# smallflyingpig/speech-to-image-translation-without-text

Hardware: AMD Instinct MI355X
Metric: StackGAN-v2 3-stage G+D train-step images/sec at 256px (higher is better)
Workload: dtype f32

## Files before the change

speech_to_image_translation_without_text_amd/csrc/s2i_conv_fwd.hip:

```cpp
#include "s2i_igemm.h"

namespace {

__global__ __launch_bounds__(256) void split_packed_kernel(const float* __restrict__ src, unsigned short* __restrict__ dst_rc,
                                                           unsigned short* __restrict__ dst_cr, int R, int C, int NP,
                                                           long long plane) {
  __shared__ float tile[32][33];
  const int t = blockIdx.z;
  const int r0 = blockIdx.y * 32, c0 = blockIdx.x * 32;
  const int tx = threadIdx.x & 31, ty = threadIdx.x >> 5;
  const float* sp = src + (size_t)t * R * C;
#pragma unroll
  for (int k = 0; k < 4; ++k) {
    const int r = r0 + ty + 8 * k, c = c0 + tx;
    tile[ty + 8 * k][tx] = (r < R && c < C) ? sp[(size_t)r * C + c] : 0.f;
  }
  __syncthreads();
#pragma unroll
  for (int k = 0; k < 4; ++k) {
    if (dst_rc) {
      const int r = r0 + ty + 8 * k, c = c0 + tx;
      if (r < R && c < C) {
        float v = tile[ty + 8 * k][tx];
        const size_t o = ((size_t)t * R + r) * C + c;
        for (int pl = 0; pl < NP; ++pl) {
          const __bf16 h = (__bf16)v;
          dst_rc[pl * plane + o] = __builtin_bit_cast(unsigned short, h);
          v -= (float)h;
        }
      }
    }
    if (dst_cr) {
      const int c = c0 + ty + 8 * k, r = r0 + tx;
      if (r < R && c < C) {
        float v = tile[tx][ty + 8 * k];
        const size_t o = ((size_t)t * C + c) * R + r;
        for (int pl = 0; pl < NP; ++pl) {
          const __bf16 h = (__bf16)v;
          dst_cr[pl * plane + o] = __builtin_bit_cast(unsigned short, h);
          v -= (float)h;
        }
      }
    }
  }
}

template <int LPP>
__global__ __launch_bounds__(256) void small_n_conv_kernel(IgemmP p) {
  extern __shared__ __attribute__((aligned(16))) float wl[];
  constexpr int PPW = 64 / LPP;
  const int tid = threadIdx.x, lane = tid & 63, wave = tid >> 6;
  const int phase = blockIdx.z;
  const int py = phase >> 1, px = phase & 1;
  int s, pad, kw;
  geom(p.kind, p.g_s, p.g_pad, p.g_kw, s, pad, kw);
  for (int e = tid; e < p.T * p.Ca; e += 256) {
    const int t = e / p.Ca, c = e - t * p.Ca;
    const int tw = tap_weight(p.kind, p.flip, p.T, t, py, px);
    f32x4 v = {0.f, 0.f, 0.f, 0.f};
    if (p.wt) {
#pragma unroll
      for (int n = 0; n < 4; ++n)
        if (n < p.N) v[n] = p.w[((size_t)tw * p.wR + n) * p.ldw + c];
    } else {
#pragma unroll
      for (int n = 0; n < 4; ++n)
        if (n < p.N && n < p.ldw) v[n] = p.w[((size_t)tw * p.wR + c) * p.ldw + n];
    }
    *reinterpret_cast<f32x4*>(wl + e * 4) = v;
  }
  __syncthreads();
  const int q = lane % LPP, pl = lane / LPP;
  const int ngroups = (p.M + PPW - 1) / PPW;
  for (int grp = blockIdx.x * 4 + wave; grp < ngroups; grp += gridDim.x * 4) {
    const int m = grp * PPW + pl;
    f32x4 acc = {0.f, 0.f, 0.f, 0.f};
    int b = 0, oy = 0, ox = 0;
    if (m < p.M) {
      b = m >> p.lgHoWo;
      const int r = m & ((1 << p.lgHoWo) - 1);
      oy = r >> p.lgWo;
      ox = r & (p.Wo - 1);
      const int by = oy * s - pad, bx = ox * s - pad;
      const unsigned mask = tap_mask(p.kind, kw, by, bx, p.H, p.W, py, px);
      const long long xo = (((long long)b * p.H + by) * p.W + bx) * p.Cx + q * 4;
      for (int t = 0; t < p.T; ++t) {
        if (!((mask >> t) & 1u)) continue;
        int dy, dx;
        tap_delta(p.kind, kw, t, py, px, dy, dx);
        const long long xe = xo + ((long long)dy * p.W + dx) * p.Cx;
        f32x4 xv;
        if (p.x16) {
          const u32x2_t h = *reinterpret_cast<const u32x2_t*>(reinterpret_cast<const unsigned short*>(p.x) + xe);
          xv = f32x4{__builtin_bit_cast(float, h[0] << 16), __builtin_bit_cast(float, h[0] & 0xffff0000u),
                     __builtin_bit_cast(float, h[1] << 16), __builtin_bit_cast(float, h[1] & 0xffff0000u)};
        } else {
          xv = *reinterpret_cast<const f32x4*>(p.x + xe);
        }
        const float* wp = wl + ((size_t)t * p.Ca + q * 4) * 4;
#pragma unroll
        for (int j = 0; j < 4; ++j) acc += xv[j] * *reinterpret_cast<const f32x4*>(wp + j * 4);
      }
    }
#pragma unroll
    for (int sft = 1; sft < LPP; sft <<= 1)
#pragma unroll
      for (int n = 0; n < 4; ++n) acc[n] += __shfl_xor(acc[n], sft);
    if (q == 0 && m < p.M) {
      long long row = m;
      if (p.kind == S2I_TCONV_K4S2) row = ((long long)b * (2 * p.Ho) + 2 * oy + py) * (2 * p.Wo) + 2 * ox + px;
      f32x4 o;
#pragma unroll
      for (int n = 0; n < 4; ++n) {
        float v = acc[n];
        if (p.bias && n < p.N) v += p.bias[n];
        if (p.act == S2I_ACT_LRELU) v = v > 0.f ? v : 0.2f * v;
        else if (p.act == S2I_ACT_TANH) v = tanhf(v);
        else if (p.act == S2I_ACT_RELU) v = fmaxf(v, 0.f);
        o[n] = v;
      }
      if (p.N == 4 && !p.y16 && (p.ldy & 3) == 0) {
        *reinterpret_cast<f32x4*>(p.y + row * p.ldy) = o;
      } else {
#pragma unroll
        for (int n = 0; n < 4; ++n) {
          if (n >= p.N) break;
          if (p.y16) reinterpret_cast<unsigned short*>(p.y)[row * p.ldy + n] = f2bf(o[n]);
          else p.y[row * p.ldy + n] = o[n];
        }
      }
    }
  }
}

__global__ void splitk_reduce_kernel(const float* __restrict__ slab, int S, long long rows, int N,
                                     const float* __restrict__ bias, int act, float* __restrict__ y,
                                     int ldy, int y16) {
  const long long total = rows * N;
  for (long long e = (long long)blockIdx.x * blockDim.x + threadIdx.x; e < total;
       e += (long long)gridDim.x * blockDim.x) {
    const long long row = e / N;
    const int n = (int)(e - row * N);
    float v = 0.f;
    for (int s = 0; s < S; ++s) v += slab[(size_t)s * total + e];
    if (bias) v += bias[n];
    if (act == S2I_ACT_LRELU) v = v > 0.f ? v : 0.2f * v;
    else if (act == S2I_ACT_TANH) v = tanhf(v);
    else if (act == S2I_ACT_RELU) v = fmaxf(v, 0.f);
    if (y16) reinterpret_cast<unsigned short*>(y)[row * ldy + n] = f2bf(v);
    else y[row * ldy + n] = v;
  }
}

__global__ __launch_bounds__(256) void splitk_reduce_stats_kernel(const float* __restrict__ slab, int S, long long rows,
                                                                  int N, float* __restrict__ y, int ldy,
                                                                  float* __restrict__ part, int nparts, int cpb,
                                                                  int ppg, long long Rg, int y16) {
  __shared__ f32x4 sh[2][256];
  const int tid = threadIdx.x;
  const int rpb = 256 / cpb;
  const int ql = tid % cpb, rl = tid / cpb;
  const int quad = blockIdx.y * cpb + ql;
  const int Q = N / 4;
  const int grp = blockIdx.x / ppg, pp = blockIdx.x - grp * ppg;
  const long long chunk = (Rg + ppg - 1) / ppg;
  const long long r0 = grp * Rg + pp * chunk;
  const long long gend = (grp + 1) * Rg < rows ? (grp + 1) * Rg : rows;
  const long long r1 = r0 + chunk < gend ? r0 + chunk : gend;
  const size_t sstride = (size_t)rows * N;
  f32x4 s0 = {0.f, 0.f, 0.f, 0.f}, s1 = {0.f, 0.f, 0.f, 0.f};
  if (quad < Q) {
    for (long long row = r0 + rl; row < r1; row += rpb) {
      const float* sp = slab + row * N + quad * 4;
      f32x4 v = *reinterpret_cast<const f32x4*>(sp);
      for (int s = 1; s < S; ++s) v += *reinterpret_cast<const f32x4*>(sp + s * sstride);
      if (y16) {
        unsigned short* yp = reinterpret_cast<unsigned short*>(y) + row * ldy + quad * 4;
        *reinterpret_cast<u32x2_t*>(yp) = u32x2_t{(unsigned)f2bf(v[0]) | ((unsigned)f2bf(v[1]) << 16),
                                                 (unsigned)f2bf(v[2]) | ((unsigned)f2bf(v[3]) << 16)};
      } else {
        *reinterpret_cast<f32x4*>(y + row * ldy + quad * 4) = v;
      }
      s0 += v;
      s1 += v * v;
    }
  }
  sh[0][tid] = s0;
  sh[1][tid] = s1;
  __syncthreads();
  if (rl == 0 && quad < Q) {
    for (int r = 1; r < rpb; ++r) {
      s0 += sh[0][r * cpb + ql];
      s1 += sh[1][r * cpb + ql];
    }
    *reinterpret_cast<f32x4*>(part + ((size_t)0 * nparts + blockIdx.x) * N + quad * 4) = s0;
    *reinterpret_cast<f32x4*>(part + ((size_t)1 * nparts + blockIdx.x) * N + quad * 4) = s1;
  }
}

}

int launch_igemm_fwd(const FwdPlan& pl, const IgemmP& p, hipStream_t st) {
  const dim3 grid(pl.gx, pl.gy, pl.gz);
  switch (pl.kernel) {
    case FWD_F32_128x128: case FWD_F32IN_128x128: launch_fwd_128x128(pl, p, grid, st); break;
    case FWD_F32_128x64: case FWD_F32IN_128x64: launch_fwd_128x64(pl, p, grid, st); break;
    case FWD_F32_128x32: case FWD_F32IN_128x32: launch_fwd_128x32(pl, p, grid, st); break;
    case FWD_F32_96x128: case FWD_F32IN_96x128: launch_fwd_96x128(pl, p, grid, st); break;
    case FWD_SPLIT_128x128: case FWD_SPLIT_128x64: case FWD_SPLIT_128x32: launch_fwd_split(pl, p, grid, st); break;
    default: S2I_FAIL("igemm_fwd: kernel %d is no matrix kernel", (int)pl.kernel);
  }
  S2I_LAUNCH_CHECK("igemm_fwd");
  return 0;
}

int launch_small_n_conv(const FwdPlan& pl, const IgemmP& p, hipStream_t st) {
  const dim3 grid(pl.gx, pl.gy, pl.gz);
  const size_t shb = (size_t)pl.T * pl.Ca * 4 * sizeof(float);
  if (pl.kernel == FWD_SMALLN_4) hipLaunchKernelGGL((small_n_conv_kernel<4>), grid, dim3(256), shb, st, p);
  else if (pl.kernel == FWD_SMALLN_8) hipLaunchKernelGGL((small_n_conv_kernel<8>), grid, dim3(256), shb, st, p);
  else hipLaunchKernelGGL((small_n_conv_kernel<16>), grid, dim3(256), shb, st, p);
  S2I_LAUNCH_CHECK("small_n_conv");
  return 0;
}

int launch_splitk_reduce(const s2i_conv_desc* d, const FwdPlan& pl, const float* bias, float* y, float* part, void* ws,
                         int y16, void* stream) {
  hipStream_t st = (hipStream_t)stream;
  if (pl.reduce == FWD_REDUCE_STATS) {
    const int Q = d->N / 4;
    int cpb = 1;
    while (cpb < Q && cpb < 256) cpb <<= 1;
    const int groups = d->groups < 1 ? 1 : d->groups;
    const int nparts = stat_parts(pl, groups);
    hipLaunchKernelGGL(splitk_reduce_stats_kernel, dim3(nparts, (Q + cpb - 1) / cpb), dim3(256), 0, st,
                       (const float*)ws, pl.splitk, pl.Mrows, d->N, y, d->ldy, part, nparts, cpb, nparts / groups,
                       pl.Mrows / groups, y16);
    S2I_LAUNCH_CHECK("splitk_reduce_stats");
    return 0;
  }
  const long long total = pl.Mrows * d->N;
  int blocks = s2i_cdiv(total, 256);
  if (blocks > 4096) blocks = 4096;
  hipLaunchKernelGGL(splitk_reduce_kernel, dim3(blocks), dim3(256), 0, st, (const float*)ws, pl.splitk,
                     pl.Mrows, d->N, bias, d->act, y, d->ldy, y16);
  S2I_LAUNCH_CHECK("splitk_reduce");
  if (pl.reduce == FWD_REDUCE_COLSTATS) return s2i_colstats(y, pl.Mrows, d->N, d->ldy, part, stat_parts(pl, 1), stream);
  return 0;
}

extern "C" int s2i_split_packed_weight(const float* packed, int T, int R, int C, int planes, unsigned short* out_rc,
                                       unsigned short* out_cr, void* stream) {
  S2I_REQUIRE(packed && (out_rc || out_cr) && T > 0 && R > 0 && C > 0 && planes >= 1 && planes <= 3,
              "split_packed_weight: bad args");
  dim3 grid(s2i_cdiv(C, 32), s2i_cdiv(R, 32), T);
  hipLaunchKernelGGL(split_packed_kernel, grid, dim3(256), 0, (hipStream_t)stream, packed, out_rc, out_cr, R, C, planes,
                     (long long)T * R * C);
  S2I_LAUNCH_CHECK("split_packed_weight");
  return 0;
}
```

speech_to_image_translation_without_text_amd/csrc/s2i_wgrad.hip:

```cpp
#include "s2i_igemm.h"

namespace {

struct WgradP {
  const float* __restrict__ a;
  const float* __restrict__ cvec;
  const float* __restrict__ g;
  float* __restrict__ slab;
  int B, H, W, Ca, Cc, Cin;
  int Ho, Wo, lgWo, lgHoWo;
  int M, N, ldg, K, T, kind;
  int cps, nchunks;
  int a16, g16;
  unsigned a_bytes, c_bytes, g_bytes;
  const float* __restrict__ a_coef;
  int a_groups, a_ipg;
};

__device__ __forceinline__ bool wgrad_col(const WgradP& p, int kcol, int kw, int& c, int& dy, int& dx) {
  c = 0;
  dy = 0;
  dx = 0;
  if (kcol >= p.K) return false;
  const int t = kcol / p.Cin;
// ... 285 lines not shown
  geom(p.kind, 1, 0, 1, s, pad, kw);
  const int acol8 = tid % ATPR, arow = tid / ATPR;
  const int bcol8 = tid % BTPR, brow = tid / BTPR;
  int c, dy, dx;
  const bool kvalid = wgrad_col(p, k0 + acol8 * 8, kw, c, dy, dx);
  const int nb = n0 + bcol8 * 8;
  const bool nvalid = nb < p.N;
  const __amdgpu_buffer_rsrc_t ra_rs = __builtin_amdgcn_make_buffer_rsrc((void*)p.a, 0, p.a_bytes, 0x00020000);
  const __amdgpu_buffer_rsrc_t rg_rs = __builtin_amdgcn_make_buffer_rsrc((void*)p.g, 0, p.g_bytes, 0x00020000);
  u32x4 ra[APASS], rb[BPASS];
  auto fetch = [&](int pc) {
#pragma unroll
    for (int q = 0; q < APASS; ++q) {
      const int m = pc * PC + arow + q * AROWS;
      int b, oy, ox;
      row_pixel(p, m, b, oy, ox);
      const int iy = oy * s - pad + dy, ix = ox * s - pad + dx;
      if constexpr (A32) {
        const bool rowok = kvalid && m < p.M && iy >= 0 && iy < p.H;
        const int o0 = ((b * p.H + iy) * p.W + ix) * 16;
        const f32x4 v0 = bload4(ra_rs, (rowok && ix >= 0 && ix < p.W) ? o0 : S2I_OOB);
        const f32x4 v1 = bload4(ra_rs, (rowok && ix + 1 >= 0 && ix + 1 < p.W) ? o0 + 16 : S2I_OOB);
        ra[q] = u32x4{(unsigned)f2bf(v0[0]) | ((unsigned)f2bf(v0[1]) << 16), (unsigned)f2bf(v0[2]) | ((unsigned)f2bf(v0[3]) << 16),
                      (unsigned)f2bf(v1[0]) | ((unsigned)f2bf(v1[1]) << 16), (unsigned)f2bf(v1[2]) | ((unsigned)f2bf(v1[3]) << 16)};
      } else {
        const bool ok = kvalid && m < p.M && iy >= 0 && iy < p.H && ix >= 0 && ix < p.W;
        ra[q] = __builtin_amdgcn_raw_buffer_load_b128(ra_rs, ok ? (((b * p.H + iy) * p.W + ix) * p.Ca + c) * 2 : S2I_OOB, 0, 0);
      }
    }
#pragma unroll
    for (int q = 0; q < BPASS; ++q) {
      const int row = brow + q * BROWS;
      const int m = pc * PC + row;
      rb[q] = __builtin_amdgcn_raw_buffer_load_b128(rg_rs, (row < PC && m < p.M && nvalid) ? (m * p.ldg + nb) * 2 : S2I_OOB, 0, 0);
    }
  };

  f32x16 acc[TM][TN];
  zero_acc(acc);

  int aad[TM][2], bad[TN][2];
  wgrad_tr_addr<TM, AROWB>(lane, wm, aad);
  wgrad_tr_addr<TN, BROWB>(lane, wn, bad);

  const int c_begin = split * p.cps;
  const int c_end = min(p.nchunks, c_begin + p.cps);
  auto stage_store = [&](unsigned char* A_, unsigned char* B_) {
#pragma unroll
    for (int q = 0; q < APASS; ++q) {
      const int row = arow + q * AROWS;
      const int sw = ((row & 3) << 2) | ((row >> 2) & 3);
      *reinterpret_cast<u32x4*>(A_ + row * AROWB + 16 * ((acol8 ^ sw) & AMASK)) = ra[q];
    }
#pragma unroll
    for (int q = 0; q < BPASS; ++q) {
      const int row = brow + q * BROWS;
      const int sw = ((row & 3) << 2) | ((row >> 2) & 3);
      if (row < PC) *reinterpret_cast<u32x4*>(B_ + row * BROWB + 16 * ((bcol8 ^ sw) & BMASK)) = rb[q];
    }
  };
  auto stage_mma = [&](const unsigned char* A_, const unsigned char* B_) {
#pragma unroll
    for (int ks = 0; ks < PC / 16; ++ks) {
      bf16x8 a[TM], b[TN];
#pragma unroll
      for (int i = 0; i < TM; ++i) a[i] = lds_tr_frag(A_ + ks * 16 * AROWB, aad[i]);
#pragma unroll
      for (int j = 0; j < TN; ++j) b[j] = lds_tr_frag(B_ + ks * 16 * BROWB, bad[j]);
#pragma unroll
      for (int i = 0; i < TM; ++i)
#pragma unroll
        for (int j = 0; j < TN; ++j)
          acc[i][j] = __builtin_amdgcn_mfma_f32_32x32x16_bf16(a[i], b[j], acc[i][j], 0, 0, 0);
    }
  };
  if (c_begin < c_end) fetch(c_begin);
  for (int pc = c_begin; pc < c_end; ++pc) {
    stage_store(As, Bs);
    __syncthreads();
    if (pc + 1 < c_end) fetch(pc + 1);
    stage_mma(As, Bs);
    __syncthreads();
  }

  store_wgrad_slab<TM, TN>(p, split, k0, n0, acc, lane, wm, wn);
}

template <int CIN, int BN, int WAVES_M, int WAVES_N, int DYS>
__global__ __launch_bounds__(64 * WAVES_M * WAVES_N, 3) void wgrad_k3_rows_kernel(WgradP p) {
  constexpr int NT = 64 * WAVES_M * WAVES_N;
  constexpr int BM = 3 * CIN * DYS, RT = BM / 32;
  constexpr int TM = RT / WAVES_M, TN = BN / (32 * WAVES_N);
  static_assert(TM * WAVES_M == RT && TN * WAVES_N * 32 == BN, "tile split");
  constexpr int LDH = CIN, LDB = BN;
  constexpr int CQ = CIN / 4, HQR = 34 * CQ, HQ = DYS * HQR;
  constexpr int HPASS = (HQ + NT - 1) / NT;
  constexpr int BROWS = NT * 4 / BN, BPASS = (32 + BROWS - 1) / BROWS;
  static_assert(BROWS * BN == NT * 4, "a pass must cover whole rows");
  __shared__ __attribute__((aligned(16))) float smem[DYS * 34 * LDH + 32 * LDB];
  float* Hs = smem;
  float* Bs = smem + DYS * 34 * LDH;
  const int tid = threadIdx.x, lane = tid & 63, wave = tid >> 6;
  const int wm = wave / WAVES_N, wn = wave % WAVES_N;
  const int dy0 = DYS == 3 ? 0 : blockIdx.x, n0 = blockIdx.y * BN, split = blockIdx.z;
  const int bcol4 = tid % (BN / 4), brow = tid / (BN / 4);
  const int nb = n0 + bcol4 * 4;
  const int gcolb = nb < p.N ? nb * 4 : S2I_OOB;
  const __amdgpu_buffer_rsrc_t ra_rs = __builtin_amdgcn_make_buffer_rsrc((void*)p.a, 0, p.a_bytes, 0x00020000);
  const __amdgpu_buffer_rsrc_t rg_rs = __builtin_amdgcn_make_buffer_rsrc((void*)p.g, 0, p.g_bytes, 0x00020000);

  f32x4 rh[HPASS], rb[BPASS];
  auto fetch = [&](int pc) {
    const int m0 = pc * 32;
    const int b = m0 >> p.lgHoWo;
    const int r = m0 & ((1 << p.lgHoWo) - 1);
    const int y = r >> p.lgWo, x0 = r & (p.W - 1);
#pragma unroll
    for (int q = 0; q < HPASS; ++q) {
      const int e = tid + q * NT;
      if (e >= HQ) continue;
      const int dyl = e / HQR, er = e - dyl * HQR;
      const int iy = y + dy0 + dyl - 1;
      const int ix = x0 - 1 + er / CQ;
      const bool ok = iy >= 0 && iy < p.H && ix >= 0 && ix < p.W;
      rh[q] = bload4(ra_rs, ok ? ((b * p.H + iy) * p.W + x0 - 1) * CIN * 4 + er * 16 : S2I_OOB);
    }
#pragma unroll
    for (int q = 0; q < BPASS; ++q) {
      const int row = brow + q * BROWS;
      if (row >= 32) continue;
      rb[q] = bload4(rg_rs, gcolb == S2I_OOB ? S2I_OOB : (m0 + row) * p.ldg * 4 + gcolb);
    }
  };

  f32x16 acc[TM][TN];
  zero_acc(acc);

  const int l31 = lane & 31, lh = lane >> 5;
  int aoff[TM];
#pragma unroll
  for (int i = 0; i < TM; ++i) {
    const int rt = wm * TM + i;
    const int dyl = rt / (3 * CIN / 32), rr = rt % (3 * CIN / 32);
    aoff[i] = dyl * 34 * LDH + (rr / (CIN / 32)) * LDH + (rr % (CIN / 32)) * 32;
  }
  const float* hp = Hs + lh * LDH + l31;
  const float* bp = Bs + lh * LDB + wn * TN * 32 + l31;

  const int c_begin = split * p.cps;
  const int c_end = min(p.nchunks, c_begin + p.cps);
  if (c_begin < c_end) fetch(c_begin);
  for (int pc = c_begin; pc < c_end; ++pc) {
#pragma unroll
    for (int q = 0; q < HPASS; ++q)
      if (tid + q * NT < HQ) *reinterpret_cast<f32x4*>(Hs + (tid + q * NT) * 4) = rh[q];
#pragma unroll
    for (int q = 0; q < BPASS; ++q)
      if (brow + q * BROWS < 32) *reinterpret_cast<f32x4*>(Bs + (brow + q * BROWS) * LDB + bcol4 * 4) = rb[q];
    __syncthreads();
    if (pc + 1 < c_end) fetch(pc + 1);
    {
      float a0[TM], b0[TN], a1[TM], b1[TN];
#pragma unroll
      for (int i = 0; i < TM; ++i) a0[i] = hp[aoff[i]];
#pragma unroll
      for (int j = 0; j < TN; ++j) b0[j] = bp[j * 32];
#pragma unroll
      for (int kk = 0; kk < 16; kk += 2) {
#pragma unroll
        for (int i = 0; i < TM; ++i) a1[i] = hp[(2 * (kk + 1)) * LDH + aoff[i]];
#pragma unroll
        for (int j = 0; j < TN; ++j) b1[j] = bp[(2 * (kk + 1)) * LDB + j * 32];
        if constexpr (TM * TN >= 4) __builtin_amdgcn_sched_barrier(0);
#pragma unroll
        for (int i = 0; i < TM; ++i)
#pragma unroll
          for (int j = 0; j < TN; ++j)
            acc[i][j] = __builtin_amdgcn_mfma_f32_32x32x2f32(a0[i], b0[j], acc[i][j], 0, 0, 0);
        if constexpr (TM * TN >= 4) __builtin_amdgcn_sched_barrier(0);
        if (kk + 2 < 16) {
#pragma unroll
          for (int i = 0; i < TM; ++i) a0[i] = hp[(2 * (kk + 2)) * LDH + aoff[i]];
#pragma unroll
          for (int j = 0; j < TN; ++j) b0[j] = bp[(2 * (kk + 2)) * LDB + j * 32];
        }
        if constexpr (TM * TN >= 4) __builtin_amdgcn_sched_barrier(0);
#pragma unroll
        for (int i = 0; i < TM; ++i)
#pragma unroll
          for (int j = 0; j < TN; ++j)
            acc[i][j] = __builtin_amdgcn_mfma_f32_32x32x2f32(a1[i], b1[j], acc[i][j], 0, 0, 0);
        if constexpr (TM * TN >= 4) __builtin_amdgcn_sched_barrier(0);
      }
    }
    __syncthreads();
  }

  store_slab<TM, TN>(p.slab + (size_t)split * p.K * p.N, p.N, acc, lane, wm, wn, n0,
                     [&](int r, long long& row) { row = dy0 * 3 * CIN + r; return true; });
}

template <int LPP>
__global__ __launch_bounds__(256) void small_n_wgrad_kernel(WgradP p) {
  constexpr int PPW = 64 / LPP;
  __shared__ f32x4 red[4][9 * LPP * 4];
  const int tid = threadIdx.x, lane = tid & 63, wave = tid >> 6;
  const int q = lane % LPP, pl = lane / LPP;
  f32x4 acc[9][4];
#pragma unroll
  for (int t = 0; t < 9; ++t)
#pragma unroll
    for (int j = 0; j < 4; ++j) acc[t][j] = f32x4{0.f, 0.f, 0.f, 0.f};
  const int ngroups = p.M / PPW;
  const int wmask = p.W - 1;
  auto load_a = [&](int m) -> f32x4 {
    if (p.a16) {
      const u32x2_t h = *reinterpret_cast<const u32x2_t*>(reinterpret_cast<const unsigned short*>(p.a) + (size_t)m * p.Ca + q * 4);
      return f32x4{__builtin_bit_cast(float, h[0] << 16), __builtin_bit_cast(float, h[0] & 0xffff0000u),
                   __builtin_bit_cast(float, h[1] << 16), __builtin_bit_cast(float, h[1] & 0xffff0000u)};
    }
    return *reinterpret_cast<const f32x4*>(p.a + (size_t)m * p.Ca + q * 4);
  };
  auto load_g = [&](int m, f32x4 (&gv)[9]) {
    const int ix = m & wmask;
    const int iy = (m >> p.lgWo) & (p.H - 1);
    const float* gp = p.g + (size_t)m * 4;
#pragma unroll
    for (int dy = 0; dy < 3; ++dy)
#pragma unroll
      for (int dx = 0; dx < 3; ++dx) {
        const int oy = iy + 1 - dy, ox = ix + 1 - dx;
        const bool ok = oy >= 0 && oy < p.H && ox >= 0 && ox < p.W;
        gv[dy * 3 + dx] = ok ? *reinterpret_cast<const f32x4*>(gp + ((1 - dy) * p.W + (1 - dx)) * 4) : f32x4{0.f, 0.f, 0.f, 0.f};
      }
  };
  auto fma9 = [&](const f32x4& av, const f32x4 (&gv)[9]) {
#pragma unroll
    for (int t = 0; t < 9; ++t)
#pragma unroll
      for (int j = 0; j < 4; ++j) acc[t][j] += av[j] * gv[t];
  };
  const int stride = gridDim.x * 4;
  int grp = blockIdx.x * 4 + wave;
  for (; grp + stride < ngroups; grp += 2 * stride) {
    const int m0 = grp * PPW + pl, m1 = (grp + stride) * PPW + pl;
    f32x4 g0[9], g1[9];
    const f32x4 av0 = load_a(m0), av1 = load_a(m1);
    load_g(m0, g0);
    load_g(m1, g1);
    fma9(av0, g0);
    fma9(av1, g1);
  }
  if (grp < ngroups) {
    const int m0 = grp * PPW + pl;
    f32x4 g0[9];
    const f32x4 av0 = load_a(m0);
    load_g(m0, g0);
    fma9(av0, g0);
  }
#pragma unroll
  for (int t = 0; t < 9; ++t)
#pragma unroll
    for (int j = 0; j < 4; ++j) {
      f32x4 v = acc[t][j];
#pragma unroll
      for (int sft = LPP; sft < 64; sft <<= 1)
#pragma unroll
        for (int n = 0; n < 4; ++n) v[n] += __shfl_xor(v[n], sft);
      if (pl == 0) red[wave][(t * LPP + q) * 4 + j] = v;
    }
  __syncthreads();
  float* outp = p.slab + (size_t)blockIdx.x * p.K * 4;
  for (int e = tid; e < 9 * LPP * 4; e += 256) {
    const f32x4 v = red[0][e] + red[1][e] + red[2][e] + red[3][e];
    *reinterpret_cast<f32x4*>(outp + (size_t)e * 4) = v;
  }
}

__global__ __launch_bounds__(256) void slab_sum_tree_kernel(float* __restrict__ slab, int S, int n4) {
  __shared__ f32x4 sh[256];
  const int tid = threadIdx.x;
  const int e = blockIdx.x * 4 + (tid & 3), sl = tid >> 2;
  f32x4 v = {0.f, 0.f, 0.f, 0.f};
  if (e < n4)
    for (int s = sl; s < S; s += 64) v += *reinterpret_cast<const f32x4*>(slab + ((size_t)s * n4 + e) * 4);
  sh[tid] = v;
  __syncthreads();
  for (int h = 32; h >= 1; h >>= 1) {
    if (sl < h) sh[tid] += sh[tid + h * 4];
    __syncthreads();
  }
  if (sl == 0 && e < n4) *reinterpret_cast<f32x4*>(slab + (size_t)e * 4) = sh[tid];
}

__global__ __launch_bounds__(256) void slab_sum_kernel(float* __restrict__ slab, int S, long long n4) {
  for (long long e = (long long)blockIdx.x * blockDim.x + threadIdx.x; e < n4;
       e += (long long)gridDim.x * blockDim.x) {
    f32x4 v = *reinterpret_cast<const f32x4*>(slab + e * 4);
    for (int s = 1; s < S; ++s) v += *reinterpret_cast<const f32x4*>(slab + ((size_t)s * n4 + e) * 4);
    *reinterpret_cast<f32x4*>(slab + e * 4) = v;
  }
}

__global__ __launch_bounds__(256) void wgrad_finish_kernel(const float* __restrict__ slab, int S, int K, int N,
                                                           int Cg, int O, int I, int Tp, int T, int swap, int fold,
                                                           int accumulate, int RT, float* __restrict__ grad,
                                                           int i_off, int I_total) {
  extern __shared__ float tile[];
  const int tid = threadIdx.x;
  const int ncols = swap ? I : O, nrows = swap ? O : I;
  const int c0 = blockIdx.x * 32, r0 = blockIdx.y * RT;
  const size_t sstride = (size_t)K * N;
  const int nload = T * RT * 32;
  for (int e = tid; e < nload; e += 256) {
    const int c_l = e & 31;
    const int r_l = (e >> 5) % RT;
    const int t = (e >> 5) / RT;
    const int c = c0 + c_l, r = r0 + r_l;
    float v = 0.f;
    if (c < ncols && r < nrows) {
      const float* sp = slab + ((size_t)t * Cg + r) * N + c;
      for (int s = 0; s < S; ++s) v += sp[s * sstride];
    }
    tile[(t * RT + r_l) * 33 + c_l] = v;
  }
  __syncthreads();
  const int nout = 32 * RT * Tp;
  for (int w = tid; w < nout; w += 256) {
    const int tapo = w % Tp;
    const int rest = w / Tp;
    int o_l, i_l, r_l, c_l;
    if (swap) { i_l = rest & 31; o_l = rest >> 5; r_l = o_l; c_l = i_l; }
    else { i_l = rest % RT; o_l = rest / RT; r_l = i_l; c_l = o_l; }
    const int o = swap ? r0 + o_l : c0 + o_l;
    const int i = swap ? c0 + i_l : r0 + i_l;
    if (o >= O || i >= I) continue;
    float v;
    if (fold) {
      const int ky = tapo / 3, kx = tapo - ky * 3;
      v = 0.f;
#pragma unroll
      for (int ay = 0; ay < 2; ++ay)
#pragma unroll
        for (int ax = 0; ax < 2; ++ax) {
          const int t = ((2 - ky) + ay) * 4 + (2 - kx) + ax;
          v += tile[(t * RT + r_l) * 33 + c_l];
        }
    } else {
      v = tile[(tapo * RT + r_l) * 33 + c_l];
    }
    float* gp = grad + ((size_t)o * I_total + i_off + i) * Tp + tapo;
    *gp = accumulate ? *gp + v : v;
  }
}

}

template <int BM, int BN, int WM, int WN>
static void launch_wgrad_split(const WgradP& p, dim3 grid, int planes, hipStream_t st) {
  if (planes == 1) hipLaunchKernelGGL((igemm_wgrad_split_kernel<BM, BN, WM, WN, 1>), grid, dim3(256), 0, st, p);
  else if (planes == 2) hipLaunchKernelGGL((igemm_wgrad_split_kernel<BM, BN, WM, WN, 2>), grid, dim3(256), 0, st, p);
  else hipLaunchKernelGGL((igemm_wgrad_split_kernel<BM, BN, WM, WN, 3>), grid, dim3(256), 0, st, p);
}

static int launch_wgrad(const s2i_wgrad_desc* d, const WgPlan& pl, const float* a, const float* cvec, const float* g,
                        float* grad_oihw, void* ws, size_t ws_bytes, void* stream, int a16, int g16, const float* a_coef) {
  S2I_REQUIRE((a || d->Ca == 0) && g && grad_oihw, "wgrad: null operand");
  S2I_REQUIRE(d->Cc == 0 || cvec != nullptr, "wgrad: cvec is null but Cc > 0");
  const size_t need = wg_workspace_bytes(pl, d->N);
  S2I_REQUIRE(ws && ws_bytes >= need, "wgrad: workspace too small (%zu < %zu)", ws_bytes, need);
  hipStream_t st = (hipStream_t)stream;
  WgradP p;
  p.a = a; p.cvec = cvec; p.g = g; p.slab = (float*)ws;
  p.B = d->B; p.H = d->H; p.W = d->W; p.Ca = d->Ca; p.Cc = d->Cc; p.Cin = pl.Cin;
  p.Ho = pl.Ho; p.Wo = pl.Wo; p.lgWo = s2i_ilog2(pl.Wo); p.lgHoWo = s2i_ilog2(pl.Ho * pl.Wo);
  p.M = pl.M; p.N = d->N; p.ldg = d->ldg; p.K = pl.K; p.T = pl.T; p.kind = d->kind;
  p.cps = pl.cps; p.nchunks = pl.nchunks;
  p.a16 = a16; p.g16 = g16;
  p.a_coef = a_coef; p.a_groups = d->a_groups < 1 ? 1 : d->a_groups; p.a_ipg = d->B / p.a_groups;
  {
    const unsigned long long ab = (unsigned long long)d->B * d->H * d->W * d->Ca * (a16 ? 2ull : 4ull);
    const unsigned long long gb = (unsigned long long)pl.M * d->ldg * (g16 ? 2ull : 4ull);
    S2I_REQUIRE(ab < 0x7ff00000ull && gb < 0x7ff00000ull, "wgrad: tensor exceeds the 2 GiB buffer-addressing window");
    p.a_bytes = (unsigned)ab; p.g_bytes = (unsigned)gb;
    p.c_bytes = (unsigned)((unsigned long long)d->B * d->Cc * 4ull);
  }
  const dim3 grid(pl.gx, pl.gy, pl.gz);
#define WG_LAUNCH(id, ...) case id: hipLaunchKernelGGL((__VA_ARGS__), grid, dim3(pl.threads), 0, st, p); break
#define WG_LAUNCH_SPLIT(id, ...) case id: launch_wgrad_split<__VA_ARGS__>(p, grid, pl.planes, st); break
  switch (pl.kernel) {
    WG_LAUNCH(WG_F32_128x128, igemm_wgrad_kernel<128, 128, 2, 2>);
    WG_LAUNCH(WG_F32_128x64, igemm_wgrad_kernel<128, 64, 2, 2>);
    WG_LAUNCH(WG_F32_128x32, igemm_wgrad_kernel<128, 32, 4, 1>);
    WG_LAUNCH(WG_F32_64x64, igemm_wgrad_kernel<64, 64, 2, 2>);
    WG_LAUNCH(WG_F32_256x128, igemm_wgrad_kernel<256, 128, 4, 2>);
    WG_LAUNCH(WG_F32_256x256, igemm_wgrad_kernel<256, 256, 4, 4>);
    WG_LAUNCH(WG_F32_96x64, igemm_wgrad_kernel<96, 64, 3, 1>);
    WG_LAUNCH(WG_F32_96x32, igemm_wgrad_kernel<96, 32, 3, 1>);
    WG_LAUNCH(WG_F32IN_128x128, igemm_wgrad_kernel<128, 128, 2, 2, true>);
    WG_LAUNCH(WG_B16_128x128, igemm_wgrad_b16_kernel<128, 128, 2, 2>);
    WG_LAUNCH(WG_B16_128x64, igemm_wgrad_b16_kernel<128, 64, 2, 2>);
    WG_LAUNCH(WG_B16_128x32, igemm_wgrad_b16_kernel<128, 32, 4, 1>);
    WG_LAUNCH(WG_B16_64x64, igemm_wgrad_b16_kernel<64, 64, 2, 2>);
    WG_LAUNCH(WG_B16_256x128, igemm_wgrad_b16_kernel<256, 128, 4, 2>);
    WG_LAUNCH(WG_B16_256x256, igemm_wgrad_b16_kernel<256, 256, 4, 4>);
    WG_LAUNCH(WG_B16D1_64x64, igemm_wgrad_b16_kernel<64, 64, 2, 2, true>);
    WG_LAUNCH_SPLIT(WG_SPLIT_128x128, 128, 128, 2, 2);
    WG_LAUNCH_SPLIT(WG_SPLIT_128x64, 128, 64, 2, 2);
    WG_LAUNCH_SPLIT(WG_SPLIT_128x32, 128, 32, 4, 1);
    WG_LAUNCH_SPLIT(WG_SPLIT_64x64, 64, 64, 2, 2);
    WG_LAUNCH(WG_ROWS3_32x64, wgrad_k3_rows_kernel<32, 64, 3, 1, 3>);
    WG_LAUNCH(WG_ROWS3_32x32, wgrad_k3_rows_kernel<32, 32, 3, 1, 3>);
    WG_LAUNCH(WG_ROWS3_64x128, wgrad_k3_rows_kernel<64, 128, 2, 2, 1>);
    WG_LAUNCH(WG_ROWS3_64x64, wgrad_k3_rows_kernel<64, 64, 2, 2, 1>);
    WG_LAUNCH(WG_ROWS3_64x32, wgrad_k3_rows_kernel<64, 32, 2, 1, 1>);
    WG_LAUNCH(WG_SMALLN_16, small_n_wgrad_kernel<4>);
    WG_LAUNCH(WG_SMALLN_32, small_n_wgrad_kernel<8>);
    WG_LAUNCH(WG_SMALLN_64, small_n_wgrad_kernel<16>);
    default: S2I_FAIL("wgrad: the plan names no kernel (%d)", (int)pl.kernel);
  }
#undef WG_LAUNCH
#undef WG_LAUNCH_SPLIT
  S2I_LAUNCH_CHECK("igemm_wgrad");
  {
    const int ncols = d->swap ? d->I : d->O, nrows = d->swap ? d->O : d->I;
    int RT = 8;
    while (RT > 1 && (long long)s2i_cdiv(ncols, 32) * s2i_cdiv(nrows, RT) < 128) RT >>= 1;
    dim3 fgrid(s2i_cdiv(ncols, 32), s2i_cdiv(nrows, RT));
    const size_t shb = (size_t)pl.T * RT * 33 * sizeof(float);
    int S = pl.slabs;
    const long long kn = (long long)pl.K * d->N;
    if (pl.kernel >= WG_SMALLN_16 || (S >= 32 && (kn % 4) == 0 && kn / 4 < (1 << 18))) {
      hipLaunchKernelGGL(slab_sum_tree_kernel, dim3(s2i_cdiv(kn / 4, 4)), dim3(256), 0, st, (float*)ws, S, (int)(kn / 4));
      S2I_LAUNCH_CHECK("slab_sum_tree");
      S = 1;
    } else if (S > 2 && (kn % 4) == 0) {
      int sb = s2i_cdiv(kn / 4, 256);
      if (sb > 4096) sb = 4096;
      hipLaunchKernelGGL(slab_sum_kernel, dim3(sb), dim3(256), 0, st, (float*)ws, S, kn / 4);
      S2I_LAUNCH_CHECK("slab_sum");
      S = 1;
    }
    hipLaunchKernelGGL(wgrad_finish_kernel, fgrid, dim3(256), shb, st, (const float*)ws, S, pl.K, d->N,
                       pl.Cin, d->O, d->I, d->KH * d->KW, pl.T, d->swap, d->fold, d->accumulate, RT, grad_oihw,
                       d->i_off, d->I_total > 0 ? d->I_total : d->I);
  }
  S2I_LAUNCH_CHECK("wgrad_finish");
  return 0;
}

static int conv_wgrad_impl(const s2i_wgrad_desc* d, int planes, const float* a, const float* cvec, const float* g,
                           float* grad_oihw, void* ws, size_t ws_bytes, void* stream, int a16 = 0, int g16 = 0, const float* a_coef = nullptr) {
  WgMode mode;
  WgPlan pl;
  if (wg_mode(a16, g16, planes, a_coef != nullptr, &mode) || plan_wgrad(d, mode, &pl)) return 1;
  return launch_wgrad(d, pl, a, cvec, g, grad_oihw, ws, ws_bytes, stream, a16, g16, a_coef);
}

extern "C" int s2i_conv_wgrad_in(const s2i_wgrad_desc* d, const float* a_raw, const float* a_coef, const float* g,
                                 float* grad_oihw, void* ws, size_t ws_bytes, void* stream) {
  S2I_REQUIRE(a_coef != nullptr, "wgrad(apply-on-load): null coefficient table");
  return conv_wgrad_impl(d, 0, a_raw, nullptr, g, grad_oihw, ws, ws_bytes, stream, 0, 0, a_coef);
}

extern "C" int s2i_conv_wgrad_dt(const s2i_wgrad_desc* d, const void* a, int a_dtype, const float* cvec, const void* g,
                                 int g_dtype, float* grad_oihw, void* ws, size_t ws_bytes, void* stream) {
  S2I_REQUIRE((a_dtype == S2I_DT_F32 || a_dtype == S2I_DT_BF16) && (g_dtype == S2I_DT_F32 || g_dtype == S2I_DT_BF16),
              "wgrad: unknown dtype");
  return conv_wgrad_impl(d, 0, (const float*)a, cvec, (const float*)g, grad_oihw, ws, ws_bytes, stream,
                         a_dtype == S2I_DT_BF16, g_dtype == S2I_DT_BF16);
}

extern "C" int s2i_conv_wgrad(const s2i_wgrad_desc* d, const float* a, const float* cvec, const float* g,
                              float* grad_oihw, void* ws, size_t ws_bytes, void* stream) {
  return conv_wgrad_impl(d, 0, a, cvec, g, grad_oihw, ws, ws_bytes, stream);
}

extern "C" int s2i_conv_wgrad_split(const s2i_wgrad_desc* d, int planes, const float* a, const float* cvec,
                                    const float* g, float* grad_oihw, void* ws, size_t ws_bytes, void* stream) {
  S2I_REQUIRE(planes >= 1 && planes <= 3, "wgrad(split): need 1 to 3 bf16 planes");
  return conv_wgrad_impl(d, planes, a, cvec, g, grad_oihw, ws, ws_bytes, stream);
}
```

Measured before the change: 781.9.

## Vectorize split-K reduce, add wide prefetching stats reduce, and tune wgrad finish

Adds a float4-vectorized split-K reduction kernel for the plain-reduce path. Adds a wider stats-reduce kernel that prefetches the first slab planes, stages reduced rows in shared memory and accumulates column sums and squares from there. Rewrites the wgrad finish kernel with templated tap counts, power-of-two index math, optional float4 slab loads and a padded per-tap shared-memory stride meant to avoid bank conflicts. All of this targets bandwidth and latency in memory-bound epilogue kernels, at the cost of more kernel variants and extra dispatch conditions.

```diff
diff --git a/speech_to_image_translation_without_text_amd/csrc/s2i_conv_fwd.hip b/speech_to_image_translation_without_text_amd/csrc/s2i_conv_fwd.hip
--- a/speech_to_image_translation_without_text_amd/csrc/s2i_conv_fwd.hip
+++ b/speech_to_image_translation_without_text_amd/csrc/s2i_conv_fwd.hip
@@ -149,6 +149,41 @@
     else if (act == S2I_ACT_RELU) v = fmaxf(v, 0.f);
     if (y16) reinterpret_cast<unsigned short*>(y)[row * ldy + n] = f2bf(v);
     else y[row * ldy + n] = v;
+  }
+}
+
+__global__ __launch_bounds__(256) void splitk_reduce_v4_kernel(const float* __restrict__ slab, int S, long long rows, int N,
+                                                               const float* __restrict__ bias, int act,
+                                                               float* __restrict__ y, int ldy, int y16, long long srow,
+                                                               int scol) {
+  const long long total = rows * N;
+  const long long e0 = ((long long)blockIdx.x * blockDim.x + threadIdx.x) * 4;
+  if (e0 >= total) return;
+  long long row = e0 / N;
+  int n = (int)(e0 - row * N);
+  for (; row < rows;) {
+    const float* sp = slab + row * N + n;
+    f32x4 v = {0.f, 0.f, 0.f, 0.f};
+    for (int s = 0; s < S; ++s) v += *reinterpret_cast<const f32x4*>(sp + (size_t)s * total);
+#pragma unroll
+    for (int j = 0; j < 4; ++j) {
+      float t = v[j];
+      if (bias) t += bias[n + j];
+      if (act == S2I_ACT_LRELU) t = t > 0.f ? t : 0.2f * t;
+      else if (act == S2I_ACT_TANH) t = tanhf(t);
+      else if (act == S2I_ACT_RELU) t = fmaxf(t, 0.f);
+      v[j] = t;
+    }
+    if (y16) {
+      unsigned short* yp = reinterpret_cast<unsigned short*>(y) + row * ldy + n;
+      *reinterpret_cast<u32x2_t*>(yp) = u32x2_t{(unsigned)f2bf(v[0]) | ((unsigned)f2bf(v[1]) << 16),
+                                               (unsigned)f2bf(v[2]) | ((unsigned)f2bf(v[3]) << 16)};
+    } else {
+      *reinterpret_cast<f32x4*>(y + row * ldy + n) = v;
+    }
+    row += srow;
+    n += scol;
+    if (n >= N) { n -= N; ++row; }
   }
 }
 
@@ -198,6 +233,92 @@
   }
 }
 
+constexpr int RS_AHEAD = 2;
+template <int RS_QB>
+__global__ __launch_bounds__(256) void splitk_reduce_stats_wide_kernel(const float* __restrict__ slab, int S,
+                                                                       long long rows, int N, float* __restrict__ y,
+                                                                       int ldy, float* __restrict__ part, int nparts,
+                                                                       int rpb, int ppg, long long Rg, int y16) {
+  constexpr int RS_RW = 256 / RS_QB, RS_ROWS = 2 * RS_RW;
+  __shared__ f32x4 vt[RS_ROWS][RS_QB];
+  __shared__ f32x4 sh[2][8 * RS_QB];
+  const int tid = threadIdx.x;
+  const int ql = tid % RS_QB, rw = tid / RS_QB;
+  const int quad = blockIdx.y * RS_QB + ql;
+  const int Q = N / 4;
+  const int grp = blockIdx.x / ppg, pp = blockIdx.x - grp * ppg;
+  const long long chunk = (Rg + ppg - 1) / ppg;
+  const long long r0 = grp * Rg + pp * chunk;
+  const long long gend = (grp + 1) * Rg < rows ? (grp + 1) * Rg : rows;
+  const long long r1 = r0 + chunk < gend ? r0 + chunk : gend;
+  const size_t sstride = (size_t)rows * N;
+  const bool colok = quad < Q;
+  const bool owner = tid < RS_QB * rpb && colok;
+  const int ahead = S < RS_AHEAD ? S : RS_AHEAD;
+  f32x4 s0 = {0.f, 0.f, 0.f, 0.f}, s1 = {0.f, 0.f, 0.f, 0.f};
+  f32x4 t[2][RS_AHEAD];
+  auto issue = [&](long long base) {
+#pragma unroll
+    for (int h = 0; h < 2; ++h) {
+      const long long row = base + rw + h * RS_RW;
+      if (colok && row < r1) {
+        const float* sp = slab + row * N + quad * 4;
+#pragma unroll
+        for (int k = 0; k < RS_AHEAD; ++k)
+          if (k < ahead) t[h][k] = *reinterpret_cast<const f32x4*>(sp + k * sstride);
+      }
+    }
+  };
+  if (r0 < r1) issue(r0);
+  for (long long base = r0; base < r1; base += RS_ROWS) {
+#pragma unroll
+    for (int h = 0; h < 2; ++h) {
+      const long long row = base + rw + h * RS_RW;
+      if (colok && row < r1) {
+        const float* sp = slab + row * N + quad * 4;
+        f32x4 v = t[h][0];
+#pragma unroll
+        for (int k = 1; k < RS_AHEAD; ++k)
+          if (k < ahead) v += t[h][k];
+        for (int s = RS_AHEAD; s < S; ++s) v += *reinterpret_cast<const f32x4*>(sp + s * sstride);
+        if (y16) {
+          unsigned short* yp = reinterpret_cast<unsigned short*>(y) + row * ldy + quad * 4;
+          *reinterpret_cast<u32x2_t*>(yp) = u32x2_t{(unsigned)f2bf(v[0]) | ((unsigned)f2bf(v[1]) << 16),
+                                                   (unsigned)f2bf(v[2]) | ((unsigned)f2bf(v[3]) << 16)};
+        } else {
+          *reinterpret_cast<f32x4*>(y + row * ldy + quad * 4) = v;
+        }
+        vt[rw + h * RS_RW][ql] = v;
+      }
+    }
+    __syncthreads();
+    if (base + RS_ROWS < r1) issue(base + RS_ROWS);
+    if (owner) {
+      const long long left = r1 - base;
+      const int jend = left < RS_ROWS ? (int)left : RS_ROWS;
+      for (int j = rw; j < jend; j += rpb) {
+        const f32x4 v = vt[j][ql];
+        s0 += v;
+        s1 += v * v;
+      }
+    }
+    __syncthreads();
+  }
+  if (owner) {
+    sh[0][tid] = s0;
+    sh[1][tid] = s1;
+  }
+  __syncthreads();
+  if (rw == 0 && colok) {
+    for (int r = 1; r < rpb; ++r) {
+      s0 += sh[0][r * RS_QB + ql];
+      s1 += sh[1][r * RS_QB + ql];
+    }
+    *reinterpret_cast<f32x4*>(part + ((size_t)0 * nparts + blockIdx.x) * N + quad * 4) = s0;
+    *reinterpret_cast<f32x4*>(part + ((size_t)1 * nparts + blockIdx.x) * N + quad * 4) = s1;
+  }
+}
+
 }
 
 int launch_igemm_fwd(const FwdPlan& pl, const IgemmP& p, hipStream_t st) {
@@ -233,17 +354,34 @@
     while (cpb < Q && cpb < 256) cpb <<= 1;
     const int groups = d->groups < 1 ? 1 : d->groups;
     const int nparts = stat_parts(pl, groups);
-    hipLaunchKernelGGL(splitk_reduce_stats_kernel, dim3(nparts, (Q + cpb - 1) / cpb), dim3(256), 0, st,
-                       (const float*)ws, pl.splitk, pl.Mrows, d->N, y, d->ldy, part, nparts, cpb, nparts / groups,
-                       pl.Mrows / groups, y16);
+    const int ppg = nparts / groups;
+    const long long Rg = pl.Mrows / groups;
+    if (cpb >= 32 && s2i_cdiv(Rg, ppg) <= 16)
+      hipLaunchKernelGGL(splitk_reduce_stats_wide_kernel<32>, dim3(nparts, (Q + 31) / 32), dim3(256), 0, st,
+                         (const float*)ws, pl.splitk, pl.Mrows, d->N, y, d->ldy, part, nparts, 256 / cpb, ppg, Rg, y16);
+    else if (cpb >= 32)
+      hipLaunchKernelGGL(splitk_reduce_stats_wide_kernel<16>, dim3(nparts, (Q + 15) / 16), dim3(256), 0, st,
+                         (const float*)ws, pl.splitk, pl.Mrows, d->N, y, d->ldy, part, nparts, 256 / cpb, ppg, Rg, y16);
+    else
+      hipLaunchKernelGGL(splitk_reduce_stats_kernel, dim3(nparts, (Q + cpb - 1) / cpb), dim3(256), 0, st,
+                         (const float*)ws, pl.splitk, pl.Mrows, d->N, y, d->ldy, part, nparts, cpb, nparts / groups,
+                         pl.Mrows / groups, y16);
     S2I_LAUNCH_CHECK("splitk_reduce_stats");
     return 0;
   }
   const long long total = pl.Mrows * d->N;
-  int blocks = s2i_cdiv(total, 256);
-  if (blocks > 4096) blocks = 4096;
-  hipLaunchKernelGGL(splitk_reduce_kernel, dim3(blocks), dim3(256), 0, st, (const float*)ws, pl.splitk,
-                     pl.Mrows, d->N, bias, d->act, y, d->ldy, y16);
+  if ((d->N & 3) == 0 && (d->ldy & 3) == 0) {
+    int blocks = s2i_cdiv(total / 4, 256);
+    if (blocks > 2048) blocks = 2048;
+    const long long stride = (long long)blocks * 256 * 4;
+    hipLaunchKernelGGL(splitk_reduce_v4_kernel, dim3(blocks), dim3(256), 0, st, (const float*)ws, pl.splitk, pl.Mrows,
+                       d->N, bias, d->act, y, d->ldy, y16, stride / d->N, (int)(stride % d->N));
+  } else {
+    int blocks = s2i_cdiv(total, 256);
+    if (blocks > 4096) blocks = 4096;
+    hipLaunchKernelGGL(splitk_reduce_kernel, dim3(blocks), dim3(256), 0, st, (const float*)ws, pl.splitk,
+                       pl.Mrows, d->N, bias, d->act, y, d->ldy, y16);
+  }
   S2I_LAUNCH_CHECK("splitk_reduce");
   if (pl.reduce == FWD_REDUCE_COLSTATS) return s2i_colstats(y, pl.Mrows, d->N, d->ldy, part, stat_parts(pl, 1), stream);
   return 0;
diff --git a/speech_to_image_translation_without_text_amd/csrc/s2i_wgrad.hip b/speech_to_image_translation_without_text_amd/csrc/s2i_wgrad.hip
--- a/speech_to_image_translation_without_text_amd/csrc/s2i_wgrad.hip
+++ b/speech_to_image_translation_without_text_amd/csrc/s2i_wgrad.hip
@@ -611,41 +611,65 @@
   }
 }
 
-__global__ __launch_bounds__(256) void wgrad_finish_kernel(const float* __restrict__ slab, int S, int K, int N,
-                                                           int Cg, int O, int I, int Tp, int T, int swap, int fold,
-                                                           int accumulate, int RT, float* __restrict__ grad,
-                                                           int i_off, int I_total) {
+struct WgFinishP {
+  const float* slab;
+  float* grad;
+  int S, K, N, Cg, O, I, Tp, T, swap, fold, accumulate, lgRT, TS, i_off, I_total;
+};
+
+template <int TP, bool V4>
+__global__ __launch_bounds__(256) void wgrad_finish_kernel(const WgFinishP p) {
   extern __shared__ float tile[];
   const int tid = threadIdx.x;
-  const int ncols = swap ? I : O, nrows = swap ? O : I;
+  const int Tp = TP > 0 ? TP : p.Tp;
+  const int lgRT = p.lgRT, RT = 1 << lgRT, TS = p.TS, N = p.N, S = p.S;
+  const int ncols = p.swap ? p.I : p.O, nrows = p.swap ? p.O : p.I;
   const int c0 = blockIdx.x * 32, r0 = blockIdx.y * RT;
-  const size_t sstride = (size_t)K * N;
-  const int nload = T * RT * 32;
-  for (int e = tid; e < nload; e += 256) {
-    const int c_l = e & 31;
-    const int r_l = (e >> 5) % RT;
-    const int t = (e >> 5) / RT;
-    const int c = c0 + c_l, r = r0 + r_l;
-    float v = 0.f;
-    if (c < ncols && r < nrows) {
-      const float* sp = slab + ((size_t)t * Cg + r) * N + c;
-      for (int s = 0; s < S; ++s) v += sp[s * sstride];
-    }
-    tile[(t * RT + r_l) * 33 + c_l] = v;
+  const size_t sstride = (size_t)p.K * N;
+  if (V4) {
+    const int nload = (p.T << lgRT) * 8;
+    for (int e = tid; e < nload; e += 256) {
+      const int c_l = (e & 7) * 4;
+      const int r_l = (e >> 3) & (RT - 1);
+      const int t = (e >> 3) >> lgRT;
+      const int c = c0 + c_l, r = r0 + r_l;
+      f32x4 v = {0.f, 0.f, 0.f, 0.f};
+      if (c < ncols && r < nrows) {
+        const float* sp = p.slab + ((size_t)t * p.Cg + r) * N + c;
+        for (int s = 0; s < S; ++s) v += *reinterpret_cast<const f32x4*>(sp + s * sstride);
+      }
+      float* tp = tile + t * TS + r_l * 33 + c_l;
+#pragma unroll
+      for (int j = 0; j < 4; ++j) tp[j] = c + j < ncols ? v[j] : 0.f;
+    }
+  } else {
+    const int nload = (p.T << lgRT) * 32;
+    for (int e = tid; e < nload; e += 256) {
+      const int c_l = e & 31;
+      const int r_l = (e >> 5) & (RT - 1);
+      const int t = (e >> 5) >> lgRT;
+      const int c = c0 + c_l, r = r0 + r_l;
+      float v = 0.f;
+      if (c < ncols && r < nrows) {
+        const float* sp = p.slab + ((size_t)t * p.Cg + r) * N + c;
+        for (int s = 0; s < S; ++s) v += sp[s * sstride];
+      }
+      tile[t * TS + r_l * 33 + c_l] = v;
+    }
   }
   __syncthreads();
   const int nout = 32 * RT * Tp;
   for (int w = tid; w < nout; w += 256) {
-    const int tapo = w % Tp;
     const int rest = w / Tp;
+    const int tapo = w - rest * Tp;
     int o_l, i_l, r_l, c_l;
-    if (swap) { i_l = rest & 31; o_l = rest >> 5; r_l = o_l; c_l = i_l; }
-    else { i_l = rest % RT; o_l = rest / RT; r_l = i_l; c_l = o_l; }
-    const int o = swap ? r0 + o_l : c0 + o_l;
-    const int i = swap ? c0 + i_l : r0 + i_l;
-    if (o >= O || i >= I) continue;
+    if (p.swap) { i_l = rest & 31; o_l = rest >> 5; r_l = o_l; c_l = i_l; }
+    else { i_l = rest & (RT - 1); o_l = rest >> lgRT; r_l = i_l; c_l = o_l; }
+    const int o = p.swap ? r0 + o_l : c0 + o_l;
+    const int i = p.swap ? c0 + i_l : r0 + i_l;
+    if (o >= p.O || i >= p.I) continue;
     float v;
-    if (fold) {
+    if (p.fold) {
       const int ky = tapo / 3, kx = tapo - ky * 3;
       v = 0.f;
 #pragma unroll
@@ -653,14 +677,30 @@
 #pragma unroll
         for (int ax = 0; ax < 2; ++ax) {
           const int t = ((2 - ky) + ay) * 4 + (2 - kx) + ax;
-          v += tile[(t * RT + r_l) * 33 + c_l];
+          v += tile[t * TS + r_l * 33 + c_l];
         }
     } else {
-      v = tile[(tapo * RT + r_l) * 33 + c_l];
-    }
-    float* gp = grad + ((size_t)o * I_total + i_off + i) * Tp + tapo;
-    *gp = accumulate ? *gp + v : v;
-  }
+      v = tile[tapo * TS + r_l * 33 + c_l];
+    }
+    float* gp = p.grad + ((size_t)o * p.I_total + p.i_off + i) * Tp + tapo;
+    *gp = p.accumulate ? *gp + v : v;
+  }
+}
+
+static int wg_finish_tap_stride(int RT, int Tp) {
+  int q = (32 + Tp / 2) / Tp;
+  if (q < 1) q = 1;
+  int ts = RT * 33;
+  while ((ts & 31) != (q & 31)) ++ts;
+  return ts;
+}
+
+template <bool V4>
+static void launch_wgrad_finish(const WgFinishP& fp, dim3 grid, size_t shb, hipStream_t st) {
+  if (fp.Tp == 9) hipLaunchKernelGGL((wgrad_finish_kernel<9, V4>), grid, dim3(256), shb, st, fp);
+  else if (fp.Tp == 16) hipLaunchKernelGGL((wgrad_finish_kernel<16, V4>), grid, dim3(256), shb, st, fp);
+  else if (fp.Tp == 1) hipLaunchKernelGGL((wgrad_finish_kernel<1, V4>), grid, dim3(256), shb, st, fp);
+  else hipLaunchKernelGGL((wgrad_finish_kernel<0, V4>), grid, dim3(256), shb, st, fp);
 }
 
 }
@@ -735,24 +775,28 @@
     const int ncols = d->swap ? d->I : d->O, nrows = d->swap ? d->O : d->I;
     int RT = 8;
     while (RT > 1 && (long long)s2i_cdiv(ncols, 32) * s2i_cdiv(nrows, RT) < 128) RT >>= 1;
+    const int Tp = d->KH * d->KW;
     dim3 fgrid(s2i_cdiv(ncols, 32), s2i_cdiv(nrows, RT));
-    const size_t shb = (size_t)pl.T * RT * 33 * sizeof(float);
-    int S = pl.slabs;
+    WgFinishP fp;
+    fp.slab = (const float*)ws; fp.grad = grad_oihw;
+    fp.S = pl.slabs; fp.K = pl.K; fp.N = d->N; fp.Cg = pl.Cin; fp.O = d->O; fp.I = d->I; fp.Tp = Tp; fp.T = pl.T;
+    fp.swap = d->swap; fp.fold = d->fold; fp.accumulate = d->accumulate; fp.lgRT = s2i_ilog2(RT);
+    fp.TS = wg_finish_tap_stride(RT, Tp); fp.i_off = d->i_off; fp.I_total = d->I_total > 0 ? d->I_total : d->I;
+    const size_t shb = (size_t)pl.T * fp.TS * sizeof(float);
     const long long kn = (long long)pl.K * d->N;
-    if (pl.kernel >= WG_SMALLN_16 || (S >= 32 && (kn % 4) == 0 && kn / 4 < (1 << 18))) {
-      hipLaunchKernelGGL(slab_sum_tree_kernel, dim3(s2i_cdiv(kn / 4, 4)), dim3(256), 0, st, (float*)ws, S, (int)(kn / 4));
+    if (pl.kernel >= WG_SMALLN_16 || (fp.S >= 32 && (kn % 4) == 0 && kn / 4 < (1 << 18))) {
+      hipLaunchKernelGGL(slab_sum_tree_kernel, dim3(s2i_cdiv(kn / 4, 4)), dim3(256), 0, st, (float*)ws, fp.S, (int)(kn / 4));
       S2I_LAUNCH_CHECK("slab_sum_tree");
-      S = 1;
-    } else if (S > 2 && (kn % 4) == 0) {
+      fp.S = 1;
+    } else if (fp.S > 2 && (kn % 4) == 0) {
       int sb = s2i_cdiv(kn / 4, 256);
       if (sb > 4096) sb = 4096;
-      hipLaunchKernelGGL(slab_sum_kernel, dim3(sb), dim3(256), 0, st, (float*)ws, S, kn / 4);
+      hipLaunchKernelGGL(slab_sum_kernel, dim3(sb), dim3(256), 0, st, (float*)ws, fp.S, kn / 4);
       S2I_LAUNCH_CHECK("slab_sum");
-      S = 1;
-    }
-    hipLaunchKernelGGL(wgrad_finish_kernel, fgrid, dim3(256), shb, st, (const float*)ws, S, pl.K, d->N,
-                       pl.Cin, d->O, d->I, d->KH * d->KW, pl.T, d->swap, d->fold, d->accumulate, RT, grad_oihw,
-                       d->i_off, d->I_total > 0 ? d->I_total : d->I);
+      fp.S = 1;
+    }
+    if ((d->N & 3) == 0 && ncols <= d->N) launch_wgrad_finish<true>(fp, fgrid, shb, st);
+    else launch_wgrad_finish<false>(fp, fgrid, shb, st);
   }
   S2I_LAUNCH_CHECK("wgrad_finish");
   return 0;
```

After: 791.1, median of 6. +1.2%, better.
